# CraigIDent/SpliSER

Measured on AMD Instinct MI355X. Metric: splice sites/sec (+ reads/sec) processed, higher is better.
Workload: dtype int32/u32 counters, f64 SSE

## Files before the change

### include/spliser.h

```cpp
#ifndef SPLISER_H
#define SPLISER_H

#include <stdint.h>

#ifdef __cplusplus
extern "C" {
#endif

#define SPL_ABI_VERSION 1

typedef enum spl_status {
    SPL_OK = 0,
    SPL_ERR_ARG = -1,
    SPL_ERR_NO_DEVICE = -2,
    SPL_ERR_HIP = -3,
    SPL_ERR_IO = -4,
    SPL_ERR_FORMAT = -5,
    SPL_ERR_RANGE = -6,
    SPL_ERR_NOMEM = -7
} spl_status;

typedef struct spl_ctx spl_ctx;
typedef struct spl_dsites spl_dsites;
typedef struct spl_dreads spl_dreads;
// ... 53 lines not shown
            const uint32_t *dbl, int beta2_cryptic, int64_t *beta2_simple, int64_t *beta2_cryptic_count,
            double *beta2_weighted, double *sse);

int spl_sites_upload(spl_ctx *ctx, const spl_sites *sites, spl_dsites **out);
void spl_sites_free(spl_ctx *ctx, spl_dsites *ds);
int spl_reads_upload(spl_ctx *ctx, const spl_reads *reads, spl_dreads **out);
int spl_reads_upload_segments(spl_ctx *ctx, int n_seg, const spl_reads *segs, const int32_t *pos_shift, spl_dreads **out);
int spl_reads_begin(spl_ctx *ctx, spl_dreads **out);
int spl_reads_begin_sized(spl_ctx *ctx, int64_t expected_reads, spl_dreads **out);
int spl_reads_add(spl_ctx *ctx, spl_dreads *dr, const spl_reads *reads, int32_t pos_shift);
int spl_reads_add2(spl_ctx *ctx, spl_dreads *dr, const spl_reads *reads, int32_t pos_shift, int64_t known_max_end);
int spl_reads_add_bam(spl_ctx *ctx, spl_dreads *dr, spl_bam *bam, int tid, int32_t pos_shift);
int spl_reads_finish(spl_ctx *ctx, spl_dreads *dr);
void spl_reads_free(spl_ctx *ctx, spl_dreads *dr);
typedef struct spl_dsoa spl_dsoa;
int spl_soa_upload(spl_ctx *ctx, int n_seg, const spl_reads *segs, spl_dsoa **out);
int spl_soa_upload2(spl_ctx *ctx, int n_seg, const spl_reads *segs, const int64_t *max_end, spl_dsoa **out);
int spl_soa_upload3(spl_ctx *ctx, int n_seg, const spl_reads *segs, const int64_t *max_end, const uint8_t *const *xs, spl_dsoa **out);
void spl_soa_free(spl_ctx *ctx, spl_dsoa *soa);
int spl_reads_add_soa(spl_ctx *ctx, spl_dreads *dr, spl_dsoa *soa, int seg, int32_t pos_shift);
int spl_reads_relayout(spl_ctx *ctx, spl_dreads *dr);
int spl_reads_has_strand(const spl_dreads *dr, int *out);
int spl_reads_layout_bytes(spl_ctx *ctx, const spl_dreads *dr, int64_t *soa_bytes_out, int64_t *record_bytes_out);
int spl_layout_timing_collect(spl_ctx *ctx, float *ms_out, int capacity, int *n_out);
int spl_pack_host(const spl_reads *reads, int n_threads, int64_t *n_chunks_out, int64_t *rec_bytes_out, int64_t *n_wide_out,
                  void *chunk_desc, void *rec, uint32_t *wide);
int spl_count_launch(spl_ctx *ctx, spl_dsites *ds, const spl_dreads *dr, const spl_opts *opts);
int spl_sse_launch(spl_ctx *ctx, spl_dsites *ds, int beta2_cryptic);
int spl_counters_download(spl_ctx *ctx, const spl_dsites *ds, uint32_t *beta1, uint32_t *beta2s_reads,
                          uint32_t *dbl);
int spl_sse_download(spl_ctx *ctx, const spl_dsites *ds, int64_t *beta2_simple,
                     int64_t *beta2_cryptic_count, double *beta2_weighted, double *sse);
int spl_count_algorithmic_bytes(const spl_dsites *ds, const spl_dreads *dr, int64_t *bytes_out);
int spl_literal_queue_size(spl_ctx *ctx, const spl_dreads *dr, int64_t *n_out);
int spl_last_launch_info(const spl_ctx *ctx, int32_t *grid_out, int32_t *block_out, int32_t *lds_bytes_out);

int spl_bam_open(const char *path, int n_threads, spl_bam **out);
int spl_bam_open_stream(const char *path, int n_threads, spl_bam **out);
int spl_bam_open_deferred(const char *path, int n_threads, spl_bam **out);
int spl_bam_set_filter(spl_bam *bam, int min_mapq, int require_flags, int exclude_flags);
int spl_bam_filter_counts(spl_bam *bam, int64_t *out2);
int spl_bam_set_aux_strand(spl_bam *bam, int on);
int spl_bam_set_flagstat(spl_bam *bam, int on);
int spl_bam_flagstat(spl_bam *bam, int64_t *out32);
int spl_flagstat_add_host(uint32_t flag, int32_t tid, int32_t next_tid, uint32_t mapq, int64_t *inout32);
int spl_bam_set_any_order(spl_bam *bam, int on);
// ... 149 lines not shown
```

### spliser_amd/csrc/spl_capi.cpp

```cpp
#include <hip/hip_runtime_api.h>
#include <hip/hip_vector_types.h>

#include <sys/mman.h>

#include <algorithm>
#include <atomic>
#include <unistd.h>
#include <cstdarg>
#include <cstdio>
#include <cstring>
#include <new>
#include <string>
#include <chrono>
#include <condition_variable>
#include <functional>
#include <memory>
#include <mutex>
#include <thread>
#include <vector>

#include "../../include/spliser.h"
#include "spl_bam.h"
#include "spl_inflate.h"
#include "spl_sort.h"
// ... 350 lines not shown
        int group = -1;
        size_t group_seg = 0;
    };
    struct Group {
        DeviceReads *src = nullptr;
        std::vector<spl_layout_seg> segs;
        uint32_t n_chunks = 0;
        char *slab = nullptr;
        spl_layout_seg *d_segs = nullptr;
        spl_layout_chunk *d_chunks = nullptr;
    };
    std::vector<Segment> segs;
    std::vector<Group> groups;
    int64_t n_reads = 0, n_cigar = 0;
    uint32_t n_chunks = 0;
    uint32_t n_slots = 0;
    uint32_t chunk_shift = SPL_CHUNK_SHIFT;
    bool fused = false;
    bool finished = false;
    char *ctl = nullptr;
    spl_chunk_meta *meta = nullptr;
    uint32_t *cost = nullptr;
    uint32_t *chunk_order = nullptr;
    spl_fused_slot *by_chunk = nullptr;
    spl_fused_slot *slots = nullptr;
    uint32_t *queue = nullptr;
    uint32_t *queue_alt = nullptr;
    uint32_t *queue_total = nullptr;
    uint32_t queue_cap = 0;
    mutable int queue_turn = 0;
    mutable bool queued_pass = false;
    mutable int64_t tail_pass = -1;
};

static inline size_t align_up(size_t v, size_t a = 256) { return (v + a - 1) / a * a; }

extern "C" int spl_device_count(int *n_out)
{
    if (!n_out) return spl_set_error(SPL_ERR_ARG, "spl_device_count: null output");
    int n = 0;
    hipError_t e = hipGetDeviceCount(&n);
    if (e != hipSuccess) { *n_out = 0; return spl_set_error(SPL_ERR_NO_DEVICE, "hipGetDeviceCount: %s", hipGetErrorString(e)); }
    *n_out = n;
    return SPL_OK;
}

static int create_ctx(int device_id, void *stream, bool use_given, spl_ctx **out)
// ... 2402 lines not shown
    if (!c || n < 0 || (n && (!keys || !perm_out))) return spl_set_error(SPL_ERR_ARG, "spl_sort_keys_device: null argument");
    if (key_bits < 1 || key_bits > 64) return spl_set_error(SPL_ERR_ARG, "spl_sort_keys_device: key_bits %d is not in 1..64", key_bits);
    if ((uint64_t)n > 0xfffffff0ull) return spl_set_error(SPL_ERR_ARG, "spl_sort_keys_device: more than 2^32 keys");
    if (n == 0) return SPL_OK;
    HIP_TRY(hipSetDevice(c->device));
    uint32_t shifts[8];
    const uint32_t n_pass = spl_dev_sort_passes((uint32_t)std::min(key_bits, 32), (uint32_t)std::max(key_bits - 32, 0), shifts);
    DevBuf d_keys[2], d_perm[2], d_work;
    for (int k = 0; k < 2; ++k) { HIP_TRY(d_keys[k].get(8 * (size_t)n, c->stream)); HIP_TRY(d_perm[k].get(4 * (size_t)n, c->stream)); }
    HIP_TRY(d_work.get(spl_dev_sort_work_bytes((uint64_t)n), c->stream));
    HIP_TRY(hipMemcpyAsync(d_keys[0].p, keys, 8 * (size_t)n, hipMemcpyHostToDevice, c->stream));
    int cur = 0;
    for (uint32_t k = 0; k < n_pass; ++k, cur ^= 1)
        HIP_TRY((hipError_t)spl_dev_launch_sort_pass(d_keys[cur].as<uint64_t>(), k ? d_perm[cur].as<uint32_t>() : nullptr, (uint64_t)n, shifts[k], d_keys[cur ^ 1].as<uint64_t>(),
                                                     d_perm[cur ^ 1].as<uint32_t>(), d_work.p, c->stream));
    HIP_TRY(hipMemcpyAsync(perm_out, d_perm[cur].p, 4 * (size_t)n, hipMemcpyDeviceToHost, c->stream));
    HIP_TRY(hipStreamSynchronize(c->stream));
    return SPL_OK;
}

static int launch_layout(spl_ctx *c, spl_dreads *d)
{
    const uint32_t chunk = 1u << d->chunk_shift;
    std::vector<spl_layout_params> lps;
    for (spl_dreads::Group &g : d->groups) {
        spl_layout_params lp;
        lp.src = spl_devreads{(const int32_t *)g.src->pos, (const uint16_t *)g.src->flag, (const uint32_t *)g.src->cig_off, (const uint32_t *)g.src->cigar};
        lp.n_rec = g.src->n_rec; lp.n_ops = g.src->n_ops;
        lp.chunks = g.d_chunks; lp.rec_base = (uint8_t *)g.slab; lp.meta = d->meta;
        const int rc0 = spl_dev_launch_layout_map(&lp.src, g.d_segs, (uint32_t)g.segs.size(), g.n_chunks, chunk, g.d_chunks, d->cost, d->by_chunk, c->stream);
        if (rc0) return spl_set_error(SPL_ERR_HIP, "layout map kernel launch: %s", hipGetErrorString((hipError_t)rc0));
        lps.push_back(lp);
    }
    if (d->n_chunks) {
        splprof::Scope prof("spl_chunk_order_kernel", c->stream, 8.0 * (double)d->n_chunks);
        const int rc = spl_dev_launch_chunk_order(d->cost, d->n_chunks, chunk, d->chunk_order, d->by_chunk, d->slots, c->stream);
        if (rc) return spl_set_error(SPL_ERR_HIP, "chunk order kernel launch: %s", hipGetErrorString((hipError_t)rc));
    }
    size_t gi = 0;
    if (d->fused) return SPL_OK;
    for (spl_dreads::Group &g : d->groups) {
        const spl_layout_params &lp = lps[gi++];
        int64_t n_reads = 0, n_ops = 0;
        for (const spl_layout_seg &ls : g.segs) n_reads += ls.n_reads;
        for (const spl_dreads::Segment &seg : d->segs) if (seg.group >= 0 && &d->groups[(size_t)seg.group] == &g) n_ops += seg.n_ops;
        const bool timed = c->k_on && (size_t)(2 * c->l_used + 1) < c->l_ev.size();
        int rc;
        {
            splprof::Scope prof("spl_layout_kernel", c->stream, 10.0 * (double)n_reads + 4.0 * (double)n_ops);
            rc = spl_dev_launch_layout(&lp, g.n_chunks, chunk, c->stream, timed ? (void *)c->l_ev[2 * c->l_used] : nullptr, timed ? (void *)c->l_ev[2 * c->l_used + 1] : nullptr);
        }
        if (timed) c->l_used++;
        if (rc) return spl_set_error(SPL_ERR_HIP, "layout kernel launch: %s", hipGetErrorString((hipError_t)rc));
    }
    return SPL_OK;
}

static bool fused_wanted()
{
    const char *e = getenv("SPL_FUSED");
    return !e || atoi(e) != 0;
}

static int finish_reads(spl_ctx *c, spl_dreads *d)
{
    if (d->finished) return SPL_OK;
    if (c->stage_timing && c->tm_pieces) {
        fprintf(stderr, "[spl_reads] %lld reads: classify %.4f s, write records %.4f s (host, %d threads); H2D %zu pieces, %.1f MB, %.3f ms in the copies = %.1f GB/s\n",
                (long long)d->n_reads, c->tm_plan_s, c->tm_emit_s, c->pack_threads, c->tm_pieces, c->tm_bytes / 1e6, c->tm_copy_ms,
                c->tm_copy_ms > 0 ? c->tm_bytes / 1e6 / c->tm_copy_ms : 0.0);
        c->tm_plan_s = c->tm_emit_s = c->tm_copy_ms = 0;
        c->tm_bytes = c->tm_pieces = 0;
    }
    if (d->n_cigar > 0xfffffff0LL) return spl_set_error(SPL_ERR_ARG, "more than 2^32 CIGAR ops in one read set: use more shards");
    auto host_now = []() { return std::chrono::duration<double>(std::chrono::steady_clock::now().time_since_epoch()).count(); };
    const double tf0 = host_now();
    bool all_device = !d->segs.empty();
    for (const spl_dreads::Segment &seg : d->segs) all_device = all_device && seg.group >= 0;
    d->fused = fused_wanted() && all_device && d->groups.size() == 1;
    const size_t n = d->n_chunks;
    const uint32_t per = spl_order_per((uint32_t)n);
    d->n_slots = 8u * per;
    const size_t shard_cap = (size_t)per << d->chunk_shift;
    size_t off = 0;
    auto take = [&](size_t bytes) { size_t o = off; off = align_up(off + bytes); return o; };
    const size_t o_meta = take(sizeof(spl_chunk_meta) * std::max<size_t>(n, 1)), o_cost = take(4 * std::max<size_t>(n, 1)), o_order = take(4 * std::max<size_t>(d->n_slots, 1));
    const size_t o_by_chunk = take(sizeof(spl_fused_slot) * std::max<size_t>(n, 1)), o_slots = take(sizeof(spl_fused_slot) * std::max<size_t>(d->n_slots, 1));
    const size_t o_total = take(4);
    const size_t o_queue = take(4 * 8 * shard_cap), o_queue_alt = take(c->tail ? 4 * 8 * shard_cap : 0);
    hipError_t e = devmem::get((void **)&d->ctl, std::max<size_t>(off, 256), 'c');
    if (e != hipSuccess) return spl_set_error(SPL_ERR_HIP, "hipMalloc(%zu) for the read set: %s", off, hipGetErrorString(e));
    d->meta = (spl_chunk_meta *)(d->ctl + o_meta);
    d->cost = (uint32_t *)(d->ctl + o_cost);
    d->chunk_order = (uint32_t *)(d->ctl + o_order);
    d->by_chunk = (spl_fused_slot *)(d->ctl + o_by_chunk);
    d->slots = (spl_fused_slot *)(d->ctl + o_slots);
    d->queue_total = (uint32_t *)(d->ctl + o_total);
    d->queue = (uint32_t *)(d->ctl + o_queue);
    d->queue_alt = c->tail ? (uint32_t *)(d->ctl + o_queue_alt) : d->queue;
    d->queue_cap = (uint32_t)shard_cap;
    const double tf_alloc = host_now() - tf0;
    hipError_t q = hipSuccess;
    std::vector<spl_chunk_meta> meta;
    std::vector<uint32_t> cost;
    bool host_segs = false;
    {
        size_t k = 0;
        for (const spl_dreads::Segment &seg : d->segs) {
            if (seg.group >= 0) { k += d->groups[(size_t)seg.group].segs[seg.group_seg].n_chunks; continue; }
            if (seg.chunks.empty()) continue;
            if (!host_segs) { meta.resize(n); cost.resize(n); host_segs = true; }
            const uint64_t rec_al = align_up((size_t)seg.rec_bytes);
            const size_t k0 = k;
            for (const splpack::ChunkDesc &cd : seg.chunks) {
                spl_chunk_meta &m = meta[k];
                m.rec = (uint64_t)(uintptr_t)seg.slab + cd.rec_off;
                m.wide = (uint64_t)(uintptr_t)seg.slab + rec_al;
                m.shift = seg.shift;
// ... 311 lines not shown
    if (c) (void)hipSetDevice(c->device);
    free_device_reads(soa->reads);
    delete soa;
}

extern "C" int spl_reads_add_soa(spl_ctx *c, spl_dreads *d, spl_dsoa *soa, int seg, int32_t pos_shift)
{
    if (!c || !d || !soa) return spl_set_error(SPL_ERR_ARG, "spl_reads_add_soa: null argument");
    DeviceReads *dev = soa->reads;
    if (seg < 0 || (size_t)seg >= dev->ref_n.size()) return spl_set_error(SPL_ERR_ARG, "spl_reads_add_soa: no segment %d", seg);
    if (dev->device != c->device) return spl_set_error(SPL_ERR_ARG, "spl_reads_add_soa: the arrays are on device %d, the context on %d", dev->device, c->device);
    HIP_TRY(hipSetDevice(c->device));
    const size_t t = (size_t)seg;
    return add_segment_device(c, d, dev, dev->ref_first[t], dev->ref_n[t], dev->ref_ops[t], pos_shift, dev->ref_n[t] && pos_shift != 0 ? dev->ref_max[t] : -1);
}

extern "C" int spl_reads_has_strand(const spl_dreads *d, int *out)
{
    if (!d || !out) return spl_set_error(SPL_ERR_ARG, "spl_reads_has_strand: null argument");
    *out = d->finished && d->fused && d->groups.size() == 1 && d->groups[0].src->xs ? 1 : 0;
    return SPL_OK;
}

extern "C" int spl_reads_layout_bytes(spl_ctx *c, const spl_dreads *d, int64_t *soa_bytes_out, int64_t *record_bytes_out)
{
    if (!c || !d || !soa_bytes_out || !record_bytes_out) return spl_set_error(SPL_ERR_ARG, "spl_reads_layout_bytes: null argument");
    if (!d->finished) return spl_set_error(SPL_ERR_ARG, "spl_reads_layout_bytes: the read set is not finished (spl_reads_finish)");
    HIP_TRY(hipSetDevice(c->device));
    int64_t soa = 0, rec = 0;
    std::vector<spl_chunk_meta> meta(d->n_chunks);
    if (d->fused) {
        for (const spl_dreads::Segment &seg : d->segs) soa += 10 * seg.n_reads + 4 * seg.n_ops;
        *soa_bytes_out = soa;
        *record_bytes_out = 0;
        return SPL_OK;
    }
    if (d->n_chunks) {
        HIP_TRY(hipMemcpyAsync(meta.data(), d->meta, sizeof(spl_chunk_meta) * d->n_chunks, hipMemcpyDeviceToHost, c->stream));
        HIP_TRY(hipStreamSynchronize(c->stream));
    }
    size_t k = 0;
    for (const spl_dreads::Segment &seg : d->segs) {
        const size_t nc = seg.group >= 0 ? d->groups[(size_t)seg.group].segs[seg.group_seg].n_chunks : seg.chunks.size();
        if (seg.group >= 0) {
            soa += 10 * seg.n_reads + 4 * seg.n_ops;
            for (size_t j = 0; j < nc; ++j) rec += (int64_t)spl_run_offset(meta[k + j].n, 4);
// ... 762 lines not shown
```

### spliser_amd/csrc/spl_devpack.h

```cpp
#ifndef SPL_DEVPACK_H
#define SPL_DEVPACK_H
#include <stdint.h>

#include "spl_pack.h"

struct spl_devreads {
    const int32_t *pos;
    const uint16_t *flag;
    const uint32_t *cig_off;
    const uint32_t *cigar;
};

struct spl_layout_seg {
    int64_t first;
    int64_t n_reads;
    uint32_t chunk0;
    uint32_t dev0;
    uint32_t n_chunks;
    int32_t shift;
};

#define SPL_LAYOUT_SLOT(chunk_reads) ((size_t)(chunk_reads) * SPL_REC_OTHER + 256u)

struct spl_layout_chunk {
// ... 16 lines not shown
    int32_t shift;
    uint32_t seg_op0;
    int32_t pos0;
    uint32_t unused0;
    uint32_t ob[SPL_FUSED_TILES_MAX + 1];
    uint32_t unused1[3];
};
static_assert(sizeof(spl_fused_slot) == 64, "one scalar load of sixteen words");

struct spl_layout_params {
    spl_devreads src;
    int64_t n_rec;
    int64_t n_ops;
    const spl_layout_chunk *chunks;
    uint8_t *rec_base;
    spl_chunk_meta *meta;
};

static inline uint32_t spl_layout_seg_chunks(int64_t first, int64_t n_reads, uint32_t chunk)
{
    return n_reads > 0 ? (uint32_t)((first + n_reads - 1) / chunk - first / chunk + 1) : 0u;
}
static inline uint32_t spl_order_per(uint32_t n_chunks) { return ((n_chunks + 7u) / 8u + 7u) / 8u * 8u; }

#ifdef __cplusplus
extern "C" {
#endif
int spl_dev_launch_layout_map(const spl_devreads *src, const spl_layout_seg *segs, uint32_t n_segs, uint32_t n_chunks, uint32_t chunk, spl_layout_chunk *chunks, uint32_t *cost,
                              spl_fused_slot *by_chunk, void *stream);
int spl_dev_launch_layout(const spl_layout_params *p, uint32_t n_dev_chunks, uint32_t chunk, void *stream, void *ev_start, void *ev_stop);
int spl_dev_launch_chunk_order(const uint32_t *cost, uint32_t n_chunks, uint32_t chunk, uint32_t *order, const spl_fused_slot *by_chunk, spl_fused_slot *slots, void *stream);
#ifdef __cplusplus
}
#endif
#endif
```

### spliser_amd/csrc/spl_devpack.hip

```cpp
#include <hip/hip_runtime.h>
#include <hip/hip_ext.h>
#include <stdint.h>

#include "spl_pack.h"
#include "spl_devpack.h"
#include "spl_layout_tile.h"

using namespace spllay;

__global__ __launch_bounds__(256) void spl_layout_map_kernel(const spl_devreads src, const spl_layout_seg *segs, uint32_t n_segs, uint32_t n_chunks, uint32_t chunk,
                                                             spl_layout_chunk *chunks, uint32_t *cost, spl_fused_slot *by_chunk)
{
    const uint32_t k = blockIdx.x * 256u + threadIdx.x;
    if (k >= n_chunks) return;
    uint32_t a = 0, b = n_segs;
    while (b - a > 1u) {
        const uint32_t mid = (a + b) >> 1;
        if (segs[mid].dev0 <= k) a = mid; else b = mid;
    }
    const spl_layout_seg s = segs[a];
    const int64_t cell = s.first / chunk + (int64_t)(k - s.dev0), c0 = cell * (int64_t)chunk, c1 = c0 + chunk;
    spl_layout_chunk c;
    c.lo = s.first > c0 ? s.first : c0;
    const int64_t hi = s.first + s.n_reads < c1 ? s.first + s.n_reads : c1;
    c.n = (uint32_t)(hi - c.lo);
    c.o_lo = src.cig_off[c.lo]; c.o_hi = src.cig_off[hi]; c.seg_op0 = src.cig_off[s.first];
    c.shift = s.shift;
    c.flat = s.chunk0 + (k - s.dev0);
    chunks[k] = c;
    cost[c.flat] = (3u * (c.o_hi - c.o_lo) + c.n) / 2u;
    spl_fused_slot f;
    f.lo = c.lo; f.chunk = c.flat; f.n = c.n; f.shift = c.shift; f.seg_op0 = c.seg_op0;
    f.pos0 = c.n ? src.pos[c.lo] : 0;
    f.unused0 = 0; f.unused1[0] = f.unused1[1] = f.unused1[2] = 0;
    const uint32_t tiles = chunk >> SPL_TILE_FUSED_SHIFT;
    for (uint32_t q = 0; q <= SPL_FUSED_TILES_MAX; ++q) {
        int64_t i = c0 + (int64_t)q * SPL_TILE_FUSED;
        i = i < c.lo ? c.lo : (i > hi ? hi : i);
        f.ob[q] = q == 0u ? c.o_lo : (q >= tiles ? c.o_hi : src.cig_off[i]);
    }
    by_chunk[c.flat] = f;
}

template <int C>
__global__ __launch_bounds__(C / 4) __attribute__((amdgpu_waves_per_eu(8, 8))) void spl_layout_kernel(const spl_layout_params p)
{
    constexpr uint32_t T = C / 4, NW = T / 64, STAGE = 4 * C;
    __shared__ uint32_t s_ops[STAGE];
    __shared__ uint32_t s_cnt[NW][2];
    __shared__ int32_t s_first;
    const uint32_t k = blockIdx.x;
    const spl_layout_chunk ch = p.chunks[k];
    uint32_t n[4];
    layout_tile<C>(p.src, p.n_rec, p.n_ops, ch, (lay_lds_w32 *)s_ops, (lay_lds_w32 *)&s_cnt[0][0], (lay_lds_i32 *)&s_first, RecordsInMemory{p.rec_base, SPL_LAYOUT_SLOT(C)}, n);
    if (threadIdx.x == 0) {
        uint8_t *const rec = p.rec_base + (size_t)k * SPL_LAYOUT_SLOT(C);
        spl_chunk_meta m;
        m.rec = (uint64_t)(uintptr_t)rec;
        m.wide = (uint64_t)(uintptr_t)(p.src.cigar + ch.seg_op0);
        m.shift = ch.shift;
        m.first_pos = s_first;
        m.n[0] = (uint16_t)n[0]; m.n[1] = (uint16_t)n[1]; m.n[2] = (uint16_t)n[2]; m.n[3] = (uint16_t)n[3];
        p.meta[ch.flat] = m;
    }
}

__global__ __launch_bounds__(1024) void spl_chunk_order_kernel(const uint32_t *cost, uint32_t n, uint32_t per, uint32_t *order, const spl_fused_slot *by_chunk,
                                                               spl_fused_slot *slots)
{
    constexpr uint32_t NB = 4096;
    __shared__ uint32_t s_hist[NB];
    __shared__ uint32_t s_part[1024];
    const uint32_t x = blockIdx.x, t = threadIdx.x;
    for (uint32_t b = t; b < NB; b += 1024u) s_hist[b] = 0;
    __syncthreads();
    auto chunk_of = [&](uint32_t e) { return (x + 8u * (e >> 3)) * 8u + (e & 7u); };
    auto key_of = [&](uint32_t c) { const uint32_t q = c >> 4; return NB - 1u - (q < NB ? q : NB - 1u); };
    for (uint32_t e = t; e < per; e += 1024u) {
        const uint32_t j = chunk_of(e);
        if (j < n) atomicAdd(&s_hist[key_of(cost[j])], 1u);
    }
    __syncthreads();
    const uint32_t h0 = s_hist[4 * t], h1 = s_hist[4 * t + 1], h2 = s_hist[4 * t + 2], h3 = s_hist[4 * t + 3];
    s_part[t] = h0 + h1 + h2 + h3;
    __syncthreads();
    for (uint32_t s = 1; s < 1024u; s <<= 1) {
        const uint32_t a = t >= s ? s_part[t - s] : 0u;
        __syncthreads();
        s_part[t] += a;
        __syncthreads();
    }
    const uint32_t before = s_part[t] - (h0 + h1 + h2 + h3), total = s_part[1023];
    __syncthreads();
    s_hist[4 * t] = before; s_hist[4 * t + 1] = before + h0; s_hist[4 * t + 2] = before + h0 + h1; s_hist[4 * t + 3] = before + h0 + h1 + h2;
    __syncthreads();
    uint32_t *const mine = order + (size_t)x * per;
    spl_fused_slot *const mine_slots = slots + (size_t)x * per;
    for (uint32_t e = t; e < per; e += 1024u) {
        const uint32_t j = chunk_of(e);
        if (j < n) {
            const uint32_t dst = atomicAdd(&s_hist[key_of(cost[j])], 1u);
            mine[dst] = j;
            const uint4 *from = (const uint4 *)(by_chunk + j);
            uint4 *to = (uint4 *)(mine_slots + dst);
            const uint4 a = from[0], b = from[1], c = from[2], d = from[3];
            to[0] = a; to[1] = b; to[2] = c; to[3] = d;
        }
    }
    for (uint32_t s = total + t; s < per; s += 1024u) {
        mine[s] = 0xffffffffu;
        uint4 *to = (uint4 *)(mine_slots + s);
        to[0] = make_uint4(0u, 0u, SPL_SLOT_EMPTY, 0u);
        to[1] = to[2] = to[3] = make_uint4(0u, 0u, 0u, 0u);
    }
}

extern "C" int spl_dev_launch_layout_map(const spl_devreads *src, const spl_layout_seg *segs, uint32_t n_segs, uint32_t n_chunks, uint32_t chunk, spl_layout_chunk *chunks,
                                         uint32_t *cost, spl_fused_slot *by_chunk, void *stream)
{
    if (!n_segs || !n_chunks) return 0;
    hipLaunchKernelGGL(spl_layout_map_kernel, dim3((n_chunks + 255u) / 256u), dim3(256), 0, (hipStream_t)stream, *src, segs, n_segs, n_chunks, chunk, chunks, cost, by_chunk);
    return (int)hipGetLastError();
}

extern "C" int spl_dev_launch_layout(const spl_layout_params *p, uint32_t n_dev_chunks, uint32_t chunk, void *stream, void *ev_start, void *ev_stop)
{
    if (!n_dev_chunks) return 0;
    hipStream_t st = (hipStream_t)stream;
    hipEvent_t e0 = (hipEvent_t)ev_start, e1 = (hipEvent_t)ev_stop;
    if (chunk == (uint32_t)SPL_CHUNK) hipExtLaunchKernelGGL(spl_layout_kernel<SPL_CHUNK>, dim3(n_dev_chunks), dim3(SPL_CHUNK / 4), 0, st, e0, e1, 0, *p);
    else if (chunk == (uint32_t)SPL_CHUNK_BIG) hipExtLaunchKernelGGL(spl_layout_kernel<SPL_CHUNK_BIG>, dim3(n_dev_chunks), dim3(SPL_CHUNK_BIG / 4), 0, st, e0, e1, 0, *p);
    else return (int)hipErrorInvalidValue;
    return (int)hipGetLastError();
}

extern "C" int spl_dev_launch_chunk_order(const uint32_t *cost, uint32_t n_chunks, uint32_t chunk, uint32_t *order, const spl_fused_slot *by_chunk, spl_fused_slot *slots,
                                          void *stream)
{
    if (!n_chunks) return 0;
    (void)chunk;
    hipLaunchKernelGGL(spl_chunk_order_kernel, dim3(8), dim3(1024), 0, (hipStream_t)stream, cost, n_chunks, spl_order_per(n_chunks), order, by_chunk, slots);
    return (int)hipGetLastError();
}
```

### spliser_amd/native.py

```python
import ctypes
import os
import subprocess

import numpy as np

HERE = os.path.dirname(os.path.abspath(__file__))
LIB_PATH = os.environ.get("SPLISER_HIP_LIB") or os.path.join(HERE, "libspliser_hip.so")
CSRC = os.path.join(HERE, "csrc")

STRANDED_CODE = {None: 0, False: 0, "": 0, "fr": 1, "rf": 2}
STRAND_FROM_XS = 3


class SpliserNativeError(RuntimeError):
    def __init__(self, code, message):
        RuntimeError.__init__(self, "libspliser_hip error %d: %s" % (code, message))
        self.code = code


class spl_sites(ctypes.Structure):
    _fields_ = [("n_sites", ctypes.c_int64), ("pos", ctypes.c_void_p), ("strand", ctypes.c_void_p),
                ("part_off", ctypes.c_void_p), ("part_pos", ctypes.c_void_p), ("part_site", ctypes.c_void_p),
                ("comp_off", ctypes.c_void_p), ("comp_pos", ctypes.c_void_p), ("alpha", ctypes.c_void_p),
                ("edge_cnt", ctypes.c_void_p)]


class spl_reads(ctypes.Structure):
    _fields_ = [("n_reads", ctypes.c_int64), ("pos", ctypes.c_void_p), ("flag", ctypes.c_void_p),
                ("cig_off", ctypes.c_void_p), ("cigar", ctypes.c_void_p)]


class spl_opts(ctypes.Structure):
    _fields_ = [("stranded", ctypes.c_int32), ("combine_mode", ctypes.c_int32), ("flags", ctypes.c_int32)]


OPT_PAIR_KERNEL = 1
OPT_WAVE_AGGREGATION = 2


EXPORTS = [
    "spl_abi_version", "spl_last_error", "spl_device_count", "spl_trim", "spl_create", "spl_create_on_stream", "spl_destroy",
    "spl_sync", "spl_pass_barrier", "spl_timer_begin", "spl_timer_end", "spl_kernel_timing_begin", "spl_kernel_timing_collect", "spl_prof_enable", "spl_prof_report", "spl_count", "spl_sse", "spl_sites_upload", "spl_sites_free",
    "spl_reads_upload", "spl_reads_upload_segments", "spl_reads_begin", "spl_reads_begin_sized", "spl_reads_add", "spl_reads_add2", "spl_reads_add_bam", "spl_reads_add_bam_share", "spl_reads_finish",
    "spl_soa_upload", "spl_soa_upload2", "spl_soa_upload3", "spl_reads_has_strand", "spl_soa_free", "spl_reads_add_soa", "spl_reads_relayout", "spl_layout_timing_collect", "spl_reads_layout_bytes",
    "spl_pack_host", "spl_reads_free", "spl_count_launch", "spl_sse_launch", "spl_counters_download",
    "spl_sse_download", "spl_count_algorithmic_bytes", "spl_literal_queue_size", "spl_last_launch_info", "spl_bam_open", "spl_bam_open_stream", "spl_bam_open_deferred", "spl_bam_set_filter", "spl_bam_set_aux_strand", "spl_bam_aux_strand", "spl_bam_aux_strand_host", "spl_bam_filter_counts", "spl_bam_set_flagstat", "spl_bam_flagstat", "spl_flagstat_add_host", "spl_bam_set_any_order", "spl_bam_any_order_sorted", "spl_sort_keys_device", "spl_bam_decode_device", "spl_bam_reserve_device", "spl_bam_share_plan", "spl_bam_share_range", "spl_bam_share_info", "spl_bam_share_count_host", "spl_bam_share_ref", "spl_bam_decode_device_share", "spl_bam_decoded_on_device", "spl_bam_wait_device", "spl_bam_start", "spl_bam_compression_ratio", "spl_bam_sample", "spl_bam_wait_ref", "spl_bam_wait_all", "spl_bam_cancel", "spl_bam_decline_reason", "spl_sam_open", "spl_bam_is_text", "spl_bam_text_compression", "spl_bam_text_blocks", "spl_bam_close",
    "spl_bam_n_ref", "spl_bam_ref_name", "spl_bam_ref_length", "spl_bam_n_records", "spl_bam_reads", "spl_bam_write", "spl_bam_write2",
    "spl_gene_search", "spl_junctions", "spl_junctions_get", "spl_junctions_stats", "spl_junction_walk_host", "spl_strand_tally", "spl_strand_rule_host", "spl_coverage", "spl_coverage_totals", "spl_coverage_download", "spl_coverage_free", "spl_coverage_rule_host", "spl_bedgraph_append", "spl_gene_count", "spl_gene_count_rule_host", "spl_simple_span_host", "spl_sites_index_info", "spl_sites_index_download", "spl_tsv_append", "spl_tsv_append_many", "spl_fmt_fixed",
    "spl_bed_open", "spl_gff_open", "spl_text_close", "spl_text_rows", "spl_text_n_chrom", "spl_text_chrom_name", "spl_text_chrom",
    "spl_text_i64", "spl_text_strand", "spl_text_names",
    "spl_combine_open", "spl_combine_close", "spl_combine_rows", "spl_combine_n_texts", "spl_combine_text", "spl_combine_region_runs",
    "spl_combine_keep_gene", "spl_combine_merge", "spl_combine_n_sites", "spl_combine_n_gap_sites", "spl_combine_skipped",
    "spl_combine_n_tables", "spl_combine_table", "spl_combine_answers", "spl_combine_write", "spl_fmt_repr",
]

_lib = None


def build(force=False):
    if force:
        subprocess.check_call(["make", "-s", "-C", CSRC, "clean"])
    subprocess.check_call(["make", "-s", "-C", CSRC])
    return LIB_PATH


def lib():
    global _lib
# ... 297 lines not shown

    def add_soa(self, soa, seg, shift=0):
        _check(lib().spl_reads_add_soa(self.ctx._h, self._h, soa._h, ctypes.c_int(int(seg)), ctypes.c_int32(int(shift))))
        self.n += soa.n[seg]

    def finish(self):
        _check(lib().spl_reads_finish(self.ctx._h, self._h))
        return self

    def has_strand(self):
        out = ctypes.c_int(0)
        _check(lib().spl_reads_has_strand(self._h, ctypes.byref(out)))
        return bool(out.value)

    def junctions_stats(self):
        b, ms = ctypes.c_int64(0), ctypes.c_float(-1.0)
        _check(lib().spl_junctions_stats(self.ctx._h, ctypes.byref(b), ctypes.byref(ms)))
        return b.value, ms.value

    def layout_bytes(self):
        a, b = ctypes.c_int64(0), ctypes.c_int64(0)
        _check(lib().spl_reads_layout_bytes(self.ctx._h, self._h, ctypes.byref(a), ctypes.byref(b)))
        return a.value, b.value

    def relayout(self):
        _check(lib().spl_reads_relayout(self.ctx._h, self._h))

    def __enter__(self):
        return self

    def __exit__(self, *exc):
        self.free()

    def literal_queue_size(self):
        out = ctypes.c_int64(0)
        _check(lib().spl_literal_queue_size(self.ctx._h, self._h, ctypes.byref(out)))
        return out.value

    def junctions(self, stranded=0, min_anchor=0, min_intron=0, max_intron=0):
        n = ctypes.c_int64(0)
        _check(lib().spl_junctions(self.ctx._h, self._h, ctypes.c_int(int(stranded)), ctypes.c_int32(int(min_anchor)),
                                   ctypes.c_int32(int(min_intron)), ctypes.c_int32(int(max_intron)), ctypes.byref(n)))
        n = n.value
        out = dict(left=np.empty(n, np.int32), right=np.empty(n, np.int32), strand=np.empty(n, np.uint8),
                   count=np.empty(n, np.uint32), anchor_left=np.empty(n, np.uint32), anchor_right=np.empty(n, np.uint32))
        _check(lib().spl_junctions_get(self.ctx._h, _ptr(out["left"]), _ptr(out["right"]), _ptr(out["strand"]), _ptr(out["count"]),
# ... 762 lines not shown
```

Measured before the change: 173.4 million.

## Fuse chunk layout mapping and cost-ordered slot construction into one parallel kernel

For fused read sets, the layout-map kernel and the 8-block chunk-order kernel are replaced by a single multi-block kernel. Each block recomputes chunk descriptors and costs directly from the read segments and scatters both slots and chunk descriptors in place. This drops the intermediate by_chunk buffer, one kernel launch, and the serial 8×1024-thread ordering. The order kernel now spreads over many 256-thread blocks, with each block redundantly tallying the cost histogram over the whole shard and using a wave-shuffle prefix scan. The price is redundant histogram work per block (extra cig_off reads in the fused path). A slot download API is also added for inspection.

```diff
diff --git a/include/spliser.h b/include/spliser.h
--- a/include/spliser.h
+++ b/include/spliser.h
@@ -99,6 +99,8 @@
 int spl_reads_relayout(spl_ctx *ctx, spl_dreads *dr);
 int spl_reads_has_strand(const spl_dreads *dr, int *out);
 int spl_reads_layout_bytes(spl_ctx *ctx, const spl_dreads *dr, int64_t *soa_bytes_out, int64_t *record_bytes_out);
+int spl_reads_slots_download(spl_ctx *ctx, const spl_dreads *dr, int64_t *n_chunks_out, int64_t *n_slots_out, int *fused_out,
+                             uint32_t *order_out, void *slots_out, void *chunks_out);
 int spl_layout_timing_collect(spl_ctx *ctx, float *ms_out, int capacity, int *n_out);
 int spl_pack_host(const spl_reads *reads, int n_threads, int64_t *n_chunks_out, int64_t *rec_bytes_out, int64_t *n_wide_out,
                   void *chunk_desc, void *rec, uint32_t *wide);
diff --git a/spliser_amd/csrc/spl_capi.cpp b/spliser_amd/csrc/spl_capi.cpp
--- a/spliser_amd/csrc/spl_capi.cpp
+++ b/spliser_amd/csrc/spl_capi.cpp
@@ -396,7 +396,6 @@
     spl_chunk_meta *meta = nullptr;
     uint32_t *cost = nullptr;
     uint32_t *chunk_order = nullptr;
-    spl_fused_slot *by_chunk = nullptr;
     spl_fused_slot *slots = nullptr;
     uint32_t *queue = nullptr;
     uint32_t *queue_alt = nullptr;
@@ -2845,23 +2844,30 @@
 static int launch_layout(spl_ctx *c, spl_dreads *d)
 {
     const uint32_t chunk = 1u << d->chunk_shift;
+    if (d->fused) {
+        spl_dreads::Group &g = d->groups[0];
+        const spl_devreads src{(const int32_t *)g.src->pos, (const uint16_t *)g.src->flag, (const uint32_t *)g.src->cig_off, (const uint32_t *)g.src->cigar};
+        splprof::Scope prof("spl_chunk_slots_kernel", c->stream, 104.0 * (double)d->n_chunks);
+        const int rc = spl_dev_launch_chunk_slots(&src, g.d_segs, (uint32_t)g.segs.size(), g.n_chunks, chunk, g.d_chunks, d->chunk_order, d->slots, c->stream);
+        if (rc) return spl_set_error(SPL_ERR_HIP, "chunk slots kernel launch: %s", hipGetErrorString((hipError_t)rc));
+        return SPL_OK;
+    }
     std::vector<spl_layout_params> lps;
     for (spl_dreads::Group &g : d->groups) {
         spl_layout_params lp;
         lp.src = spl_devreads{(const int32_t *)g.src->pos, (const uint16_t *)g.src->flag, (const uint32_t *)g.src->cig_off, (const uint32_t *)g.src->cigar};
         lp.n_rec = g.src->n_rec; lp.n_ops = g.src->n_ops;
         lp.chunks = g.d_chunks; lp.rec_base = (uint8_t *)g.slab; lp.meta = d->meta;
-        const int rc0 = spl_dev_launch_layout_map(&lp.src, g.d_segs, (uint32_t)g.segs.size(), g.n_chunks, chunk, g.d_chunks, d->cost, d->by_chunk, c->stream);
+        const int rc0 = spl_dev_launch_layout_map(&lp.src, g.d_segs, (uint32_t)g.segs.size(), g.n_chunks, chunk, g.d_chunks, d->cost, c->stream);
         if (rc0) return spl_set_error(SPL_ERR_HIP, "layout map kernel launch: %s", hipGetErrorString((hipError_t)rc0));
         lps.push_back(lp);
     }
     if (d->n_chunks) {
-        splprof::Scope prof("spl_chunk_order_kernel", c->stream, 8.0 * (double)d->n_chunks);
-        const int rc = spl_dev_launch_chunk_order(d->cost, d->n_chunks, chunk, d->chunk_order, d->by_chunk, d->slots, c->stream);
+        splprof::Scope prof("spl_chunk_slots_kernel", c->stream, 8.0 * (double)d->n_chunks);
+        const int rc = spl_dev_launch_chunk_order(d->cost, d->n_chunks, d->chunk_order, c->stream);
         if (rc) return spl_set_error(SPL_ERR_HIP, "chunk order kernel launch: %s", hipGetErrorString((hipError_t)rc));
     }
     size_t gi = 0;
-    if (d->fused) return SPL_OK;
     for (spl_dreads::Group &g : d->groups) {
         const spl_layout_params &lp = lps[gi++];
         int64_t n_reads = 0, n_ops = 0;
@@ -2908,7 +2914,7 @@
     size_t off = 0;
     auto take = [&](size_t bytes) { size_t o = off; off = align_up(off + bytes); return o; };
     const size_t o_meta = take(sizeof(spl_chunk_meta) * std::max<size_t>(n, 1)), o_cost = take(4 * std::max<size_t>(n, 1)), o_order = take(4 * std::max<size_t>(d->n_slots, 1));
-    const size_t o_by_chunk = take(sizeof(spl_fused_slot) * std::max<size_t>(n, 1)), o_slots = take(sizeof(spl_fused_slot) * std::max<size_t>(d->n_slots, 1));
+    const size_t o_slots = take(sizeof(spl_fused_slot) * std::max<size_t>(d->n_slots, 1));
     const size_t o_total = take(4);
     const size_t o_queue = take(4 * 8 * shard_cap), o_queue_alt = take(c->tail ? 4 * 8 * shard_cap : 0);
     hipError_t e = devmem::get((void **)&d->ctl, std::max<size_t>(off, 256), 'c');
@@ -2916,7 +2922,6 @@
     d->meta = (spl_chunk_meta *)(d->ctl + o_meta);
     d->cost = (uint32_t *)(d->ctl + o_cost);
     d->chunk_order = (uint32_t *)(d->ctl + o_order);
-    d->by_chunk = (spl_fused_slot *)(d->ctl + o_by_chunk);
     d->slots = (spl_fused_slot *)(d->ctl + o_slots);
     d->queue_total = (uint32_t *)(d->ctl + o_total);
     d->queue = (uint32_t *)(d->ctl + o_queue);
@@ -3274,6 +3279,24 @@
     return SPL_OK;
 }
 
+extern "C" int spl_reads_slots_download(spl_ctx *c, const spl_dreads *d, int64_t *n_chunks_out, int64_t *n_slots_out, int *fused_out, uint32_t *order_out, void *slots_out,
+                                        void *chunks_out)
+{
+    if (!c || !d) return spl_set_error(SPL_ERR_ARG, "spl_reads_slots_download: null argument");
+    if (!d->finished) return spl_set_error(SPL_ERR_ARG, "spl_reads_slots_download: the read set is not finished (spl_reads_finish)");
+    if (n_chunks_out) *n_chunks_out = (int64_t)d->n_chunks;
+    if (n_slots_out) *n_slots_out = (int64_t)d->n_slots;
+    if (fused_out) *fused_out = d->fused ? 1 : 0;
+    if (!d->n_chunks || (!order_out && !slots_out && !chunks_out)) return SPL_OK;
+    if ((slots_out || chunks_out) && !d->fused) return spl_set_error(SPL_ERR_ARG, "spl_reads_slots_download: only a fused read set has slots and one list of chunk descriptors");
+    HIP_TRY(hipSetDevice(c->device));
+    if (order_out) HIP_TRY(hipMemcpyAsync(order_out, d->chunk_order, 4 * (size_t)d->n_slots, hipMemcpyDeviceToHost, c->stream));
+    if (slots_out) HIP_TRY(hipMemcpyAsync(slots_out, d->slots, sizeof(spl_fused_slot) * (size_t)d->n_slots, hipMemcpyDeviceToHost, c->stream));
+    if (chunks_out) HIP_TRY(hipMemcpyAsync(chunks_out, d->groups[0].d_chunks, sizeof(spl_layout_chunk) * (size_t)d->n_chunks, hipMemcpyDeviceToHost, c->stream));
+    HIP_TRY(hipStreamSynchronize(c->stream));
+    return SPL_OK;
+}
+
 extern "C" int spl_reads_layout_bytes(spl_ctx *c, const spl_dreads *d, int64_t *soa_bytes_out, int64_t *record_bytes_out)
 {
     if (!c || !d || !soa_bytes_out || !record_bytes_out) return spl_set_error(SPL_ERR_ARG, "spl_reads_layout_bytes: null argument");
diff --git a/spliser_amd/csrc/spl_devpack.h b/spliser_amd/csrc/spl_devpack.h
--- a/spliser_amd/csrc/spl_devpack.h
+++ b/spliser_amd/csrc/spl_devpack.h
@@ -62,14 +62,17 @@
     return n_reads > 0 ? (uint32_t)((first + n_reads - 1) / chunk - first / chunk + 1) : 0u;
 }
 static inline uint32_t spl_order_per(uint32_t n_chunks) { return ((n_chunks + 7u) / 8u + 7u) / 8u * 8u; }
+#define SPL_ORDER_CHUNKS_MAX 0xfff00000u
 
 #ifdef __cplusplus
 extern "C" {
 #endif
 int spl_dev_launch_layout_map(const spl_devreads *src, const spl_layout_seg *segs, uint32_t n_segs, uint32_t n_chunks, uint32_t chunk, spl_layout_chunk *chunks, uint32_t *cost,
-                              spl_fused_slot *by_chunk, void *stream);
+                              void *stream);
 int spl_dev_launch_layout(const spl_layout_params *p, uint32_t n_dev_chunks, uint32_t chunk, void *stream, void *ev_start, void *ev_stop);
-int spl_dev_launch_chunk_order(const uint32_t *cost, uint32_t n_chunks, uint32_t chunk, uint32_t *order, const spl_fused_slot *by_chunk, spl_fused_slot *slots, void *stream);
+int spl_dev_launch_chunk_slots(const spl_devreads *src, const spl_layout_seg *segs, uint32_t n_segs, uint32_t n_chunks, uint32_t chunk, spl_layout_chunk *chunks, uint32_t *order,
+                               spl_fused_slot *slots, void *stream);
+int spl_dev_launch_chunk_order(const uint32_t *cost, uint32_t n_chunks, uint32_t *order, void *stream);
 #ifdef __cplusplus
 }
 #endif
diff --git a/spliser_amd/csrc/spl_devpack.hip b/spliser_amd/csrc/spl_devpack.hip
--- a/spliser_amd/csrc/spl_devpack.hip
+++ b/spliser_amd/csrc/spl_devpack.hip
@@ -8,8 +8,18 @@
 
 using namespace spllay;
 
+__device__ __forceinline__ void chunk_reads(const spl_layout_seg &s, uint32_t i, uint32_t sh, int64_t &c0, int64_t &lo, int64_t &hi)
+{
+    c0 = ((s.first >> sh) + (int64_t)i) << sh;
+    const int64_t c1 = c0 + ((int64_t)1 << sh), end = s.first + s.n_reads;
+    lo = s.first > c0 ? s.first : c0;
+    hi = end < c1 ? end : c1;
+}
+
+__device__ __forceinline__ uint32_t chunk_cost(uint32_t ops, uint32_t reads) { return (3u * ops + reads) / 2u; }
+
 __global__ __launch_bounds__(256) void spl_layout_map_kernel(const spl_devreads src, const spl_layout_seg *segs, uint32_t n_segs, uint32_t n_chunks, uint32_t chunk,
-                                                             spl_layout_chunk *chunks, uint32_t *cost, spl_fused_slot *by_chunk)
+                                                             spl_layout_chunk *chunks, uint32_t *cost)
 {
     const uint32_t k = blockIdx.x * 256u + threadIdx.x;
     if (k >= n_chunks) return;
@@ -19,27 +29,15 @@
         if (segs[mid].dev0 <= k) a = mid; else b = mid;
     }
     const spl_layout_seg s = segs[a];
-    const int64_t cell = s.first / chunk + (int64_t)(k - s.dev0), c0 = cell * (int64_t)chunk, c1 = c0 + chunk;
+    int64_t c0, hi;
     spl_layout_chunk c;
-    c.lo = s.first > c0 ? s.first : c0;
-    const int64_t hi = s.first + s.n_reads < c1 ? s.first + s.n_reads : c1;
+    chunk_reads(s, k - s.dev0, (uint32_t)__builtin_ctz(chunk), c0, c.lo, hi);
     c.n = (uint32_t)(hi - c.lo);
     c.o_lo = src.cig_off[c.lo]; c.o_hi = src.cig_off[hi]; c.seg_op0 = src.cig_off[s.first];
     c.shift = s.shift;
     c.flat = s.chunk0 + (k - s.dev0);
     chunks[k] = c;
-    cost[c.flat] = (3u * (c.o_hi - c.o_lo) + c.n) / 2u;
-    spl_fused_slot f;
-    f.lo = c.lo; f.chunk = c.flat; f.n = c.n; f.shift = c.shift; f.seg_op0 = c.seg_op0;
-    f.pos0 = c.n ? src.pos[c.lo] : 0;
-    f.unused0 = 0; f.unused1[0] = f.unused1[1] = f.unused1[2] = 0;
-    const uint32_t tiles = chunk >> SPL_TILE_FUSED_SHIFT;
-    for (uint32_t q = 0; q <= SPL_FUSED_TILES_MAX; ++q) {
-        int64_t i = c0 + (int64_t)q * SPL_TILE_FUSED;
-        i = i < c.lo ? c.lo : (i > hi ? hi : i);
-        f.ob[q] = q == 0u ? c.o_lo : (q >= tiles ? c.o_hi : src.cig_off[i]);
-    }
-    by_chunk[c.flat] = f;
+    cost[c.flat] = chunk_cost(c.o_hi - c.o_lo, c.n);
 }
 
 template <int C>
@@ -65,61 +63,157 @@
     }
 }
 
-__global__ __launch_bounds__(1024) void spl_chunk_order_kernel(const uint32_t *cost, uint32_t n, uint32_t per, uint32_t *order, const spl_fused_slot *by_chunk,
-                                                               spl_fused_slot *slots)
-{
-    constexpr uint32_t NB = 4096;
-    __shared__ uint32_t s_hist[NB];
-    __shared__ uint32_t s_part[1024];
-    const uint32_t x = blockIdx.x, t = threadIdx.x;
-    for (uint32_t b = t; b < NB; b += 1024u) s_hist[b] = 0;
-    __syncthreads();
-    auto chunk_of = [&](uint32_t e) { return (x + 8u * (e >> 3)) * 8u + (e & 7u); };
+#define SPL_SLOTS_SEGS_LDS 256u
+template <bool FUSED>
+__global__ __launch_bounds__(256) void spl_chunk_slots_kernel(const spl_devreads src, const spl_layout_seg *segs, uint32_t n_segs, const uint32_t *cost, uint32_t n, uint32_t per,
+                                                              uint32_t chunk, spl_layout_chunk *chunks, uint32_t *order, spl_fused_slot *slots)
+{
+    constexpr uint32_t NB = 4096, T = 256, U = 4, NONE = 0xffffffffu;
+    __shared__ alignas(16) uint32_t s_hist[NB];
+    __shared__ alignas(16) uint32_t s_key[T];
+    __shared__ uint32_t s_wave[T / 64];
+    __shared__ spl_layout_seg s_segs[FUSED ? SPL_SLOTS_SEGS_LDS : 1u];
+    const uint32_t x = blockIdx.x & 7u, t = threadIdx.x, e0 = (blockIdx.x >> 3) * T, e = e0 + t;
+    const uint32_t sh = (uint32_t)__builtin_ctz(chunk);
+    const bool staged = n_segs <= SPL_SLOTS_SEGS_LDS;
+    for (uint32_t b = t; b < NB; b += T) s_hist[b] = 0;
+    if (FUSED && staged)
+        for (uint32_t i = t; i < n_segs; i += T) s_segs[i] = segs[i];
+    __syncthreads();
+    auto chunk_of = [&](uint32_t f) { return (x + 8u * (f >> 3)) * 8u + (f & 7u); };
     auto key_of = [&](uint32_t c) { const uint32_t q = c >> 4; return NB - 1u - (q < NB ? q : NB - 1u); };
-    for (uint32_t e = t; e < per; e += 1024u) {
-        const uint32_t j = chunk_of(e);
-        if (j < n) atomicAdd(&s_hist[key_of(cost[j])], 1u);
-    }
-    __syncthreads();
-    const uint32_t h0 = s_hist[4 * t], h1 = s_hist[4 * t + 1], h2 = s_hist[4 * t + 2], h3 = s_hist[4 * t + 3];
-    s_part[t] = h0 + h1 + h2 + h3;
-    __syncthreads();
-    for (uint32_t s = 1; s < 1024u; s <<= 1) {
-        const uint32_t a = t >= s ? s_part[t - s] : 0u;
-        __syncthreads();
-        s_part[t] += a;
-        __syncthreads();
-    }
-    const uint32_t before = s_part[t] - (h0 + h1 + h2 + h3), total = s_part[1023];
-    __syncthreads();
-    s_hist[4 * t] = before; s_hist[4 * t + 1] = before + h0; s_hist[4 * t + 2] = before + h0 + h1; s_hist[4 * t + 3] = before + h0 + h1 + h2;
-    __syncthreads();
-    uint32_t *const mine = order + (size_t)x * per;
-    spl_fused_slot *const mine_slots = slots + (size_t)x * per;
-    for (uint32_t e = t; e < per; e += 1024u) {
-        const uint32_t j = chunk_of(e);
-        if (j < n) {
-            const uint32_t dst = atomicAdd(&s_hist[key_of(cost[j])], 1u);
-            mine[dst] = j;
-            const uint4 *from = (const uint4 *)(by_chunk + j);
-            uint4 *to = (uint4 *)(mine_slots + dst);
-            const uint4 a = from[0], b = from[1], c = from[2], d = from[3];
-            to[0] = a; to[1] = b; to[2] = c; to[3] = d;
-        }
-    }
-    for (uint32_t s = total + t; s < per; s += 1024u) {
-        mine[s] = 0xffffffffu;
-        uint4 *to = (uint4 *)(mine_slots + s);
-        to[0] = make_uint4(0u, 0u, SPL_SLOT_EMPTY, 0u);
-        to[1] = to[2] = to[3] = make_uint4(0u, 0u, 0u, 0u);
+    auto seg_of = [&](uint32_t j) {
+        uint32_t a = 0, b = n_segs;
+        while (b - a > 1u) {
+            const uint32_t mid = (a + b) >> 1;
+            if ((staged ? s_segs[mid].chunk0 : segs[mid].chunk0) <= j) a = mid; else b = mid;
+        }
+        return staged ? s_segs[a] : segs[a];
+    };
+    auto tally = [&](uint32_t f0, uint32_t f1) {
+        for (uint32_t f = f0 + t; f < f1; f += U * T) {
+            uint32_t c[U];
+            bool is[U];
+            if constexpr (FUSED) {
+                uint32_t o_lo[U], o_hi[U], reads[U];
+#pragma unroll
+                for (uint32_t u = 0; u < U; ++u) {
+                    const uint32_t j = chunk_of(f + u * T);
+                    is[u] = f + u * T < f1 && j < n;
+                    o_lo[u] = o_hi[u] = reads[u] = 0;
+                    if (is[u]) {
+                        const spl_layout_seg s = seg_of(j);
+                        int64_t c0, lo, hi;
+                        chunk_reads(s, j - s.chunk0, sh, c0, lo, hi);
+                        o_lo[u] = src.cig_off[lo]; o_hi[u] = src.cig_off[hi]; reads[u] = (uint32_t)(hi - lo);
+                    }
+                }
+#pragma unroll
+                for (uint32_t u = 0; u < U; ++u) c[u] = chunk_cost(o_hi[u] - o_lo[u], reads[u]);
+            } else {
+#pragma unroll
+                for (uint32_t u = 0; u < U; ++u) {
+                    const uint32_t j = chunk_of(f + u * T);
+                    is[u] = f + u * T < f1 && j < n;
+                    c[u] = is[u] ? cost[j] : 0u;
+                }
+            }
+#pragma unroll
+            for (uint32_t u = 0; u < U; ++u)
+                if (is[u]) atomicAdd(&s_hist[key_of(c[u])], 1u);
+        }
+    };
+    const uint32_t j = chunk_of(e);
+    const bool is_chunk = e < per && j < n;
+    uint32_t key = NONE;
+    spl_layout_chunk c = {};
+    spl_fused_slot fs = {};
+    uint32_t k = 0;
+    if (is_chunk) {
+        if constexpr (FUSED) {
+            const spl_layout_seg s = seg_of(j);
+            int64_t c0, hi;
+            chunk_reads(s, j - s.chunk0, sh, c0, c.lo, hi);
+            k = s.dev0 + (j - s.chunk0);
+            c.n = (uint32_t)(hi - c.lo);
+            c.o_lo = src.cig_off[c.lo]; c.o_hi = src.cig_off[hi]; c.seg_op0 = src.cig_off[s.first];
+            c.shift = s.shift;
+            c.flat = j;
+            fs.lo = c.lo; fs.chunk = c.flat; fs.n = c.n; fs.shift = c.shift; fs.seg_op0 = c.seg_op0;
+            fs.pos0 = c.n ? src.pos[c.lo] : 0;
+            fs.unused0 = 0; fs.unused1[0] = fs.unused1[1] = fs.unused1[2] = 0;
+            const uint32_t tiles = chunk >> SPL_TILE_FUSED_SHIFT;
+#pragma unroll
+            for (uint32_t q = 0; q <= SPL_FUSED_TILES_MAX; ++q) {
+                int64_t i = c0 + (int64_t)q * SPL_TILE_FUSED;
+                i = i < c.lo ? c.lo : (i > hi ? hi : i);
+                fs.ob[q] = q == 0u ? c.o_lo : (q >= tiles ? c.o_hi : src.cig_off[i]);
+            }
+            key = key_of(chunk_cost(c.o_hi - c.o_lo, c.n));
+        } else
+            key = key_of(cost[j]);
+    }
+    s_key[t] = key;
+    tally(0u, e0);
+    __syncthreads();
+    uint32_t before = is_chunk ? s_hist[key] : 0u;
+    __syncthreads();
+    if (is_chunk) atomicAdd(&s_hist[key], 1u);
+    tally(e0 + T < per ? e0 + T : per, per);
+    for (uint32_t u = 0; u < (t | 63u) + 1u; u += 4u) {
+        const uint4 q = *(const uint4 *)&s_key[u];
+        before += (q.x == key && u < t) + (q.y == key && u + 1u < t) + (q.z == key && u + 2u < t) + (q.w == key && u + 3u < t);
+    }
+    __syncthreads();
+    uint4 h[4];
+    uint32_t sum = 0;
+#pragma unroll
+    for (uint32_t i = 0; i < 4u; ++i) {
+        h[i] = *(const uint4 *)&s_hist[16u * t + 4u * i];
+        sum += h[i].x + h[i].y + h[i].z + h[i].w;
+    }
+    uint32_t incl = sum;
+#pragma unroll
+    for (uint32_t s = 1; s < 64u; s <<= 1) {
+        const uint32_t up = (uint32_t)__shfl_up((int)incl, s, 64);
+        if ((t & 63u) >= s) incl += up;
+    }
+    if ((t & 63u) == 63u) s_wave[t >> 6] = incl;
+    __syncthreads();
+    uint32_t run = incl - sum;
+    for (uint32_t w = 0; w < (t >> 6); ++w) run += s_wave[w];
+#pragma unroll
+    for (uint32_t i = 0; i < 4u; ++i) {
+        uint4 o;
+        o.x = run; o.y = run + h[i].x; o.z = o.y + h[i].y; o.w = o.z + h[i].z;
+        run = o.w + h[i].w;
+        *(uint4 *)&s_hist[16u * t + 4u * i] = o;
+    }
+    __syncthreads();
+    if (e >= per) return;
+    const size_t slot = (size_t)x * per + (is_chunk ? s_hist[key] + before : e);
+    if (is_chunk) {
+        order[slot] = j;
+        if constexpr (FUSED) {
+            chunks[k] = c;
+            slots[slot] = fs;
+        }
+    } else {
+        order[slot] = NONE;
+        if constexpr (FUSED) {
+            uint4 *to = (uint4 *)(slots + slot);
+            to[0] = make_uint4(0u, 0u, SPL_SLOT_EMPTY, 0u);
+            to[1] = to[2] = to[3] = make_uint4(0u, 0u, 0u, 0u);
+        }
     }
 }
 
 extern "C" int spl_dev_launch_layout_map(const spl_devreads *src, const spl_layout_seg *segs, uint32_t n_segs, uint32_t n_chunks, uint32_t chunk, spl_layout_chunk *chunks,
-                                         uint32_t *cost, spl_fused_slot *by_chunk, void *stream)
+                                         uint32_t *cost, void *stream)
 {
     if (!n_segs || !n_chunks) return 0;
-    hipLaunchKernelGGL(spl_layout_map_kernel, dim3((n_chunks + 255u) / 256u), dim3(256), 0, (hipStream_t)stream, *src, segs, n_segs, n_chunks, chunk, chunks, cost, by_chunk);
+    if (chunk & (chunk - 1u)) return (int)hipErrorInvalidValue;
+    hipLaunchKernelGGL(spl_layout_map_kernel, dim3((n_chunks + 255u) / 256u), dim3(256), 0, (hipStream_t)stream, *src, segs, n_segs, n_chunks, chunk, chunks, cost);
     return (int)hipGetLastError();
 }
 
@@ -134,11 +228,23 @@
     return (int)hipGetLastError();
 }
 
-extern "C" int spl_dev_launch_chunk_order(const uint32_t *cost, uint32_t n_chunks, uint32_t chunk, uint32_t *order, const spl_fused_slot *by_chunk, spl_fused_slot *slots,
-                                          void *stream)
+static dim3 chunk_slots_grid(uint32_t n_chunks) { return dim3(8u * ((spl_order_per(n_chunks) + 255u) / 256u)); }
+
+extern "C" int spl_dev_launch_chunk_slots(const spl_devreads *src, const spl_layout_seg *segs, uint32_t n_segs, uint32_t n_chunks, uint32_t chunk, spl_layout_chunk *chunks,
+                                          uint32_t *order, spl_fused_slot *slots, void *stream)
+{
+    if (!n_segs || !n_chunks) return 0;
+    if ((chunk & (chunk - 1u)) || n_chunks > SPL_ORDER_CHUNKS_MAX) return (int)hipErrorInvalidValue;
+    hipLaunchKernelGGL(spl_chunk_slots_kernel<true>, chunk_slots_grid(n_chunks), dim3(256), 0, (hipStream_t)stream, *src, segs, n_segs, (const uint32_t *)nullptr, n_chunks,
+                       spl_order_per(n_chunks), chunk, chunks, order, slots);
+    return (int)hipGetLastError();
+}
+
+extern "C" int spl_dev_launch_chunk_order(const uint32_t *cost, uint32_t n_chunks, uint32_t *order, void *stream)
 {
     if (!n_chunks) return 0;
-    (void)chunk;
-    hipLaunchKernelGGL(spl_chunk_order_kernel, dim3(8), dim3(1024), 0, (hipStream_t)stream, cost, n_chunks, spl_order_per(n_chunks), order, by_chunk, slots);
-    return (int)hipGetLastError();
-}
+    if (n_chunks > SPL_ORDER_CHUNKS_MAX) return (int)hipErrorInvalidValue;
+    hipLaunchKernelGGL(spl_chunk_slots_kernel<false>, chunk_slots_grid(n_chunks), dim3(256), 0, (hipStream_t)stream, spl_devreads{}, (const spl_layout_seg *)nullptr, 0u, cost,
+                       n_chunks, spl_order_per(n_chunks), 1u, (spl_layout_chunk *)nullptr, order, (spl_fused_slot *)nullptr);
+    return (int)hipGetLastError();
+}
diff --git a/spliser_amd/native.py b/spliser_amd/native.py
--- a/spliser_amd/native.py
+++ b/spliser_amd/native.py
@@ -42,7 +42,7 @@
     "spl_abi_version", "spl_last_error", "spl_device_count", "spl_trim", "spl_create", "spl_create_on_stream", "spl_destroy",
     "spl_sync", "spl_pass_barrier", "spl_timer_begin", "spl_timer_end", "spl_kernel_timing_begin", "spl_kernel_timing_collect", "spl_prof_enable", "spl_prof_report", "spl_count", "spl_sse", "spl_sites_upload", "spl_sites_free",
     "spl_reads_upload", "spl_reads_upload_segments", "spl_reads_begin", "spl_reads_begin_sized", "spl_reads_add", "spl_reads_add2", "spl_reads_add_bam", "spl_reads_add_bam_share", "spl_reads_finish",
-    "spl_soa_upload", "spl_soa_upload2", "spl_soa_upload3", "spl_reads_has_strand", "spl_soa_free", "spl_reads_add_soa", "spl_reads_relayout", "spl_layout_timing_collect", "spl_reads_layout_bytes",
+    "spl_soa_upload", "spl_soa_upload2", "spl_soa_upload3", "spl_reads_has_strand", "spl_soa_free", "spl_reads_add_soa", "spl_reads_relayout", "spl_layout_timing_collect", "spl_reads_layout_bytes", "spl_reads_slots_download",
     "spl_pack_host", "spl_reads_free", "spl_count_launch", "spl_sse_launch", "spl_counters_download",
     "spl_sse_download", "spl_count_algorithmic_bytes", "spl_literal_queue_size", "spl_last_launch_info", "spl_bam_open", "spl_bam_open_stream", "spl_bam_open_deferred", "spl_bam_set_filter", "spl_bam_set_aux_strand", "spl_bam_aux_strand", "spl_bam_aux_strand_host", "spl_bam_filter_counts", "spl_bam_set_flagstat", "spl_bam_flagstat", "spl_flagstat_add_host", "spl_bam_set_any_order", "spl_bam_any_order_sorted", "spl_sort_keys_device", "spl_bam_decode_device", "spl_bam_reserve_device", "spl_bam_share_plan", "spl_bam_share_range", "spl_bam_share_info", "spl_bam_share_count_host", "spl_bam_share_ref", "spl_bam_decode_device_share", "spl_bam_decoded_on_device", "spl_bam_wait_device", "spl_bam_start", "spl_bam_compression_ratio", "spl_bam_sample", "spl_bam_wait_ref", "spl_bam_wait_all", "spl_bam_cancel", "spl_bam_decline_reason", "spl_sam_open", "spl_bam_is_text", "spl_bam_text_compression", "spl_bam_text_blocks", "spl_bam_close",
     "spl_bam_n_ref", "spl_bam_ref_name", "spl_bam_ref_length", "spl_bam_n_records", "spl_bam_reads", "spl_bam_write", "spl_bam_write2",
@@ -386,6 +386,19 @@
         a, b = ctypes.c_int64(0), ctypes.c_int64(0)
         _check(lib().spl_reads_layout_bytes(self.ctx._h, self._h, ctypes.byref(a), ctypes.byref(b)))
         return a.value, b.value
+
+    def slots(self):
+        n, ns, fused = ctypes.c_int64(0), ctypes.c_int64(0), ctypes.c_int(0)
+        _check(lib().spl_reads_slots_download(self.ctx._h, self._h, ctypes.byref(n), ctypes.byref(ns), ctypes.byref(fused), None, None, None))
+        n, ns, fused = n.value, ns.value, bool(fused.value)
+        order = np.zeros(max(ns, 1), np.uint32)
+        slots = np.zeros((max(ns, 1), 64), np.uint8) if fused else None
+        chunks = np.zeros((max(n, 1), 32), np.uint8) if fused else None
+        _check(lib().spl_reads_slots_download(self.ctx._h, self._h, None, None, None, _ptr(order), _ptr(slots), _ptr(chunks)))
+        out = dict(fused=fused, order=order[:ns].reshape(8, ns // 8))
+        if fused:
+            out.update(slots=slots[:ns].reshape(8, ns // 8, 64), chunks=chunks[:n])
+        return out
 
     def relayout(self):
         _check(lib().spl_reads_relayout(self.ctx._h, self._h))
```

Measured after the change: 175.5 million, median of 6. 1.01x the previous value.
